# lRomul/ball-action-spotting

Measured on AMD Instinct MI355X. Metric: frame-windows/sec (fwd+bwd) at 15x736x1280, batch 4, higher is better.
Workload: dtype bf16; 1 GPU; sampling_weights_001: 4x15x736x1280 windows/GPU, fwd + focal loss + bwd + grad all-reduce + AdamW (mds.train fused focal loss / multi-tensor optimizer); global_batch=4, parallelism=dp1

## Files before the change

ball-action-spotting_amd/csrc/k_pw.hip:

```cpp
#include <stdlib.h>
#include "gemm.h"

#define PW_BM 128
#ifndef MDS_PW_GPRE3
#define MDS_PW_GPRE3 1
#endif
#define PW_BN 128
#define PW_SP 72

template <typename T> struct PwCfg;
template <> struct PwCfg<bf16_t> { static const int KC = 64, LD = 80; };
template <> struct PwCfg<float> { static const int KC = 32, LD = 40; };

template <typename T, int PRO, int WN, int BM, int TAIL, bool SPLIT = false, bool DEEP = false>
__global__ __launch_bounds__(256, (WN == 2 && BM == 128) || TAIL == 1 || SPLIT || DEEP ? 2 : 3) void pw_fwd_kernel(mds_pw_fwd_args a) {
  MDS_CHAIN_PRIO();
  static_assert(!DEEP || (TAIL != 1 && (PRO == MDS_PRO_NONE || PRO == MDS_PRO_GATE) && WN == 2 && BM == 64), "DEEP variants");
  static_assert(!SPLIT || (TAIL != 1 && (PRO == MDS_PRO_NONE || PRO == MDS_PRO_GATE) && WN == 2 && BM == 64), "SPLIT variants");
  constexpr bool POST = TAIL == 1, EPI = TAIL == 2;
  typedef typename Frag<T>::type frag_t;
  typedef Mma<T, EPI && sizeof(T) == 4 && MDS_EVAL_X3> MM;
  constexpr int KC = PwCfg<T>::KC, LD = PwCfg<T>::LD, VPR = KC / 8, RPP = 256 / VPR, NL = BM / RPP;
  constexpr int BN = 64 * WN, MFW = (WN == 2 ? BM / 32 : BM / 64), NLW = BN / RPP;
  MDS_DYN_SMEM(smem);
  T* xs = (T*)smem;
  T* ws = xs + BM * LD;
  constexpr bool STG = sizeof(T) == 2;
  T* stg = ws + BN * LD + (threadIdx.x >> 6) * 16 * PW_SP;

  const int tid = threadIdx.x, lane = tid & 63, wave = MDS_UNIFORM(tid >> 6);
  const int i = lane & 15, q = lane >> 4;
  const int wm = WN == 2 ? wave >> 1 : wave, wn = WN == 2 ? wave & 1 : 0;
  const long m0 = (long)blockIdx.x * BM;
  const int N = a.N;
  const int K = a.K;
  const int kper = SPLIT ? ((K + (int)gridDim.z * PwCfg<T>::KC - 1) / ((int)gridDim.z * PwCfg<T>::KC)) * PwCfg<T>::KC : K;
  const int KB = SPLIT ? (int)blockIdx.z * kper : 0;
  const int KE = SPLIT ? (KB + kper < K ? KB + kper : K) : K;
  const T* x = (const T*)a.x;
  const T* w = (const T*)a.w;
  T* y = (T*)a.y;
  const int svec = tid % VPR, srow = tid / VPR;
  int grow[NL];
  if (PRO == MDS_PRO_BN_SILU_GATE || PRO == MDS_PRO_GATE) {
    const long rpg = a.pro.rows_per_group;
#pragma unroll
    for (int l = 0; l < NL; ++l) {
      const long m = m0 + srow + RPP * l;
      grow[l] = (int)((m < a.M ? m : a.M - 1) / rpg);
    }
  }

  const T* xrow[NL];
  bool xok[NL];
#pragma unroll
  for (int l = 0; l < NL; ++l) {
    const long m = m0 + srow + RPP * l;
    xok[l] = m < a.M;
    xrow[l] = x + (xok[l] ? m : 0) * K + 8 * svec;
  }
  for (int n0 = blockIdx.y * BN; n0 < N; n0 += gridDim.y * BN) {
    int nfr = (N - n0 - 64 * wn) >> 4;
    nfr = nfr < 0 ? 0 : (nfr > 4 ? 4 : nfr);
    f32x4 acc[MFW][4];
#pragma unroll
    for (int mf = 0; mf < MFW; ++mf)
#pragma unroll
      for (int nf = 0; nf < 4; ++nf) acc[mf][nf] = (f32x4){0.f, 0.f, 0.f, 0.f};

    RawV4<T> rys[POST ? MFW : 1][4];
    float pb[4] = {0.f, 0.f, 0.f, 0.f};
    if (EPI && tid < BN && n0 + tid < N) { pb[0] = a.epi.scale[n0 + tid]; pb[1] = a.epi.shift[n0 + tid]; }
    if (POST) {
      if (tid < BN && n0 + tid < N) {
#pragma unroll
        for (int k = 0; k < 4; ++k) pb[k] = a.post.bn[(long)k * N + n0 + tid];
      }
      const int nfr_ = (N - n0 - 64 * wn) >> 4;
#pragma unroll
      for (int mf = 0; mf < (POST ? MFW : 1); ++mf) {
        const long m = m0 + 16 * MFW * wm + 16 * mf + i;
        const T* ysrow = (const T*)a.post.y + (m < a.M ? m : 0) * N + n0 + (nfr_ > 0 ? 64 * wn : 0) + 4 * q;
#pragma unroll
        for (int nf = 0; nf < 4; ++nf) rys[mf][nf].ld(ysrow + (nf < nfr_ ? 16 * nf : 0));
      }
    }

    constexpr int NS = DEEP ? 2 : 1;
    RawV8<T> rx[NS][NL], rw[NS][NLW];
    constexpr bool GATED = PRO == MDS_PRO_BN_SILU_GATE || PRO == MDS_PRO_GATE;
    constexpr bool GPRE = (PRO == MDS_PRO_GATE || (PRO == MDS_PRO_BN_SILU_GATE && MDS_PW_GPRE3)) && NL <= 2;
    float rg[NS][GPRE ? NL : 1][8];
    const T* wrow[NLW];
    bool wok[NLW];
#pragma unroll
    for (int l = 0; l < NLW; ++l) {
      const int n = n0 + srow + RPP * l;
      wok[l] = n < N;
      wrow[l] = w + (long)(wok[l] ? n : 0) * K + 8 * svec;
    }
    constexpr bool SPRE = PRO == MDS_PRO_BN_SILU_GATE && MDS_PW_GPRE3 && NL <= 2;
    float psc[SPRE ? 8 : 1], psh[SPRE ? 8 : 1];
    auto issue = [&](int kc, RawV8<T> (&tx)[NL], RawV8<T> (&tw)[NLW], float (&tg)[GPRE ? NL : 1][8]) {
      const bool kok = kc + 8 * svec < KE;
      if (DEEP) {
        const int ko = kok ? kc : -8 * svec;
#pragma unroll
        for (int l = 0; l < NL; ++l) {
          tx[l].ld(xrow[l] + ko);
          if (GPRE) load8f(a.pro.gate + (long)grow[l] * K + (kok ? kc + 8 * svec : 0), tg[l]);
        }
#pragma unroll
        for (int l = 0; l < NLW; ++l) tw[l].ld(wrow[l] + ko);
        return;
      }
      if (SPRE) {
        const int kp = kok ? kc + 8 * svec : 0;
        load8f(a.pro.scale + kp, (float (&)[8])psc); load8f(a.pro.shift + kp, (float (&)[8])psh);
      }
#pragma unroll
      for (int l = 0; l < NL; ++l) {
        if (xok[l] && kok) tx[l].ld(xrow[l] + kc); else tx[l].zero();
        if (GPRE) load8f(a.pro.gate + (long)grow[l] * K + (kok ? kc + 8 * svec : 0), tg[l]);
      }
#pragma unroll
      for (int l = 0; l < NLW; ++l) {
        if (wok[l] && kok) tw[l].ld(wrow[l] + kc); else tw[l].zero();
      }
    };
    auto chunk = [&](int kc, RawV8<T> (&tx)[NL], RawV8<T> (&tw)[NLW], float (&tg)[GPRE ? NL : 1][8]) {
      const int kk = kc + 8 * svec;
      const bool kin = kk < KE;
      __syncthreads();
      if (PRO == MDS_PRO_NONE) {
#pragma unroll
        for (int l = 0; l < NL; ++l) {
          if (DEEP && !(xok[l] && kin)) tx[l].zero();
          tx[l].st(xs + (srow + RPP * l) * LD + 8 * svec);
        }
      } else {
        float sc[8], sh[8];
        if (SPRE) {
#pragma unroll
          for (int j = 0; j < 8; ++j) { sc[j] = psc[SPRE ? j : 0]; sh[j] = psh[SPRE ? j : 0]; }
        } else if (PRO != MDS_PRO_GATE && kin) { load8f(a.pro.scale + kk, sc); load8f(a.pro.shift + kk, sh); }
#pragma unroll
        for (int l = 0; l < NL; ++l) {
          const int r = srow + RPP * l;
          const long m = m0 + r;
          float v[8];
          tx[l].get(v);
          if (m < a.M && kin) {
            if (PRO != MDS_PRO_GATE) {
#pragma unroll
              for (int j = 0; j < 8; ++j) {
                float z = v[j] * sc[j] + sh[j];
                v[j] = (PRO == MDS_PRO_AFFINE) ? z : siluf_(z);
              }
            }
            if (GPRE) {
#pragma unroll
              for (int j = 0; j < 8; ++j) v[j] *= tg[l][j];
            } else if (GATED) {
              float g[8];
              load8f(a.pro.gate + (long)grow[l] * K + kk, g);
#pragma unroll
              for (int j = 0; j < 8; ++j) v[j] *= g[j];
            }
          } else if (DEEP) {
#pragma unroll
            for (int j = 0; j < 8; ++j) v[j] = 0.f;
          }
          store8(xs + r * LD + 8 * svec, v);
        }
      }
#pragma unroll
      for (int l = 0; l < NLW; ++l) {
        if (DEEP && !(wok[l] && kin)) tw[l].zero();
        tw[l].st(ws + (srow + RPP * l) * LD + 8 * svec);
      }
      __syncthreads();
      if (DEEP) issue(kc + 2 * KC, tx, tw, tg);
      else if (kc + KC < KE) issue(kc + KC, tx, tw, tg);
      const int ksteps = (KE - kc >= KC) ? KC / 32 : ((KE - kc + 31) >> 5);
#pragma unroll
      for (int ks = 0; ks < KC / 32; ++ks) {
        if (DEEP || ks < ksteps) {
          typename MM::frag xf[MFW];
#pragma unroll
          for (int mf = 0; mf < MFW; ++mf) xf[mf] = MM::prep(ld_frag(xs + (16 * MFW * wm + 16 * mf + i) * LD + 32 * ks + 8 * q));
#pragma unroll
          for (int nf = 0; nf < 4; ++nf) {
            const typename MM::frag wf = MM::prep(ld_frag(ws + (64 * wn + 16 * nf + i) * LD + 32 * ks + 8 * q));
#pragma unroll
            for (int mf = 0; mf < MFW; ++mf) MM::mma(wf, xf[mf], acc[mf][nf]);
          }
        }
      }
    };
    if (!SPLIT || KB < KE) issue(KB, rx[0], rw[0], rg[0]);
    if (DEEP) {
      issue(KB + KC, rx[NS - 1], rw[NS - 1], rg[NS - 1]);
      for (int kc = KB; kc < KE; kc += 2 * KC) {
        chunk(kc, rx[0], rw[0], rg[0]);
        chunk(kc + KC, rx[NS - 1], rw[NS - 1], rg[NS - 1]);
      }
    } else {
      for (int kc = KB; kc < KE; kc += KC) chunk(kc, rx[0], rw[0], rg[0]);
    }
    if (SPLIT) {
      const long MN = a.M * (long)N;
#pragma unroll
      for (int mf = 0; mf < MFW; ++mf) {
        const long m = m0 + 16 * MFW * wm + 16 * mf + i;
        if (m < a.M) {
          float* prow = a.split_part + (long)blockIdx.z * MN + m * N + n0 + 64 * wn + 4 * q;
#pragma unroll
          for (int nf = 0; nf < 4; ++nf)
            if (nf < nfr) st_coherent4(prow + 16 * nf, acc[mf][nf]);
        }
      }
      int* lastp = (int*)smem;
      mds_wait_stores();
      __syncthreads();
      if (tid == 0) {
        int* tk = a.split_ticket + ((long)blockIdx.x * ((N + BN - 1) / BN) + n0 / BN) * MDS_PW_SPLIT_TICKET_STRIDE;
        const int t = atomicAdd(tk, 1);
        const int last = t == (int)gridDim.z - 1;
        if (last) atomicExch(tk, 0);
        *lastp = last;
      }
      __syncthreads();
      const bool last = *lastp != 0;
      __syncthreads();
      if (!last) continue;
#pragma unroll
      for (int mf = 0; mf < MFW; ++mf)
#pragma unroll
        for (int nf = 0; nf < 4; ++nf) acc[mf][nf] = (f32x4){0.f, 0.f, 0.f, 0.f};
      for (int z0 = 0; z0 < (int)gridDim.z; z0 += 4) {
        f32x4 t[4][MFW][4];
#pragma unroll
        for (int zz = 0; zz < 4; ++zz)
#pragma unroll
          for (int mf = 0; mf < MFW; ++mf) {
            const long m = m0 + 16 * MFW * wm + 16 * mf + i;
            const bool ok = m < a.M && z0 + zz < (int)gridDim.z;
            const float* prow = a.split_part + (long)(z0 + zz) * MN + m * N + n0 + 64 * wn + 4 * q;
#pragma unroll
            for (int nf = 0; nf < 4; ++nf) t[zz][mf][nf] = (ok && nf < nfr) ? ld_coherent4(prow + 16 * nf) : (f32x4){0.f, 0.f, 0.f, 0.f};
          }
#pragma unroll
        for (int zz = 0; zz < 4; ++zz)
#pragma unroll
          for (int mf = 0; mf < MFW; ++mf)
#pragma unroll
            for (int nf = 0; nf < 4; ++nf) acc[mf][nf] += t[zz][mf][nf];
      }
    }

    float ps[16], pss[16];
#pragma unroll
    for (int e = 0; e < 16; ++e) { ps[e] = 0.f; pss[e] = 0.f; }
    float* pbn = (float*)smem;
    if (POST) {
      __syncthreads();
      if (tid < BN) {
#pragma unroll
        for (int k = 0; k < 4; ++k) pbn[k * BN + tid] = pb[k];
      }
      __syncthreads();
    }
    if (EPI) {
      __syncthreads();
      if (tid < BN) { pbn[tid] = pb[0]; pbn[BN + tid] = pb[1]; }
      __syncthreads();
    }
#pragma unroll
    for (int mf = 0; mf < MFW; ++mf) {
      const long m = m0 + 16 * MFW * wm + 16 * mf + i;
      const bool ok = m < a.M;
      T* yrow = y + (ok ? m : 0) * N + n0 + 64 * wn + 4 * q;
      float v[4][4];
#pragma unroll
      for (int nf = 0; nf < 4; ++nf)
#pragma unroll
        for (int r = 0; r < 4; ++r) v[nf][r] = acc[mf][nf][r];
      if (EPI) {
#pragma unroll
        for (int nf = 0; nf < 4; ++nf) {
          const float* pc = pbn + 64 * wn + 16 * nf + 4 * q;
          const f32x4 sc = *(const f32x4*)pc, sh = *(const f32x4*)(pc + BN);
#pragma unroll
          for (int r = 0; r < 4; ++r) {
            const float z = v[nf][r] * sc[r] + sh[r];
            v[nf][r] = a.epi.mode == MDS_EPI_BN_SILU ? siluf_(z) : z;
          }
        }
      }
      if (a.residual && ok) {
        const T* rrow = (const T*)a.residual + m * N + n0 + 64 * wn + 4 * q;
#pragma unroll
        for (int nf = 0; nf < 4; ++nf) {
          if (nf < nfr) {
            float rr[4];
            load4(rrow + 16 * nf, rr);
#pragma unroll
            for (int r = 0; r < 4; ++r) v[nf][r] += rr[r];
          }
        }
      }
      if (POST) {
        const float mk = (a.post.mode == MDS_POST_MASK) ? a.post.mask[(unsigned)(ok ? m : 0) / (unsigned)a.post.rows_per_group] : 1.0f;
#pragma unroll
        for (int nf = 0; nf < 4; ++nf) {
          if (nf < nfr) {
            const float ys[4] = {rys[mf][nf].get(0), rys[mf][nf].get(1), rys[mf][nf].get(2), rys[mf][nf].get(3)};
            const float* pc = pbn + 64 * wn + 16 * nf + 4 * q;
            const f32x4 mu = *(const f32x4*)(pc + 2 * BN), rs = *(const f32x4*)(pc + 3 * BN);
            if (a.post.mode == MDS_POST_SILU) {
              const f32x4 sc = *(const f32x4*)pc, sh = *(const f32x4*)(pc + BN);
#pragma unroll
              for (int r = 0; r < 4; ++r) v[nf][r] *= silu_gradf_(ys[r] * sc[r] + sh[r]);
            }
#pragma unroll
            for (int r = 0; r < 4; ++r) {
              const float g = Elem<T>::rnd(v[nf][r]) * mk;
              ps[nf * 4 + r] += g;
              pss[nf * 4 + r] += g * ((ys[r] - mu[r]) * rs[r]);
            }
          }
        }
      }
      if (STG) {
#pragma unroll
        for (int nf = 0; nf < 4; ++nf) store4(stg + i * PW_SP + 16 * nf + 4 * q, v[nf]);
        wave_lds_sync();
        T* ybase = y + (m0 + 16 * MFW * wm + 16 * mf) * N + n0 + 64 * wn;
#pragma unroll
        for (int t = 0; t < 2; ++t) {
          const int vv = lane + 64 * t, row = vv >> 3, c = vv & 7;
          if (m0 + 16 * MFW * wm + 16 * mf + row < a.M && (c >> 1) < nfr) {
            RawV8<T> o;
            o.ld(stg + row * PW_SP + 8 * c);
            o.st(ybase + (long)row * N + 8 * c);
          }
        }
        wave_lds_sync();
      } else if (ok) {
#pragma unroll
        for (int nf = 0; nf < 4; ++nf)
          if (nf < nfr) store4(yrow + 16 * nf, v[nf]);
      }
      if (!POST) {
#pragma unroll
        for (int nf = 0; nf < 4; ++nf)
#pragma unroll
          for (int r = 0; r < 4; ++r) { ps[nf * 4 + r] += v[nf][r]; pss[nf * 4 + r] += v[nf][r] * v[nf][r]; }
      }
    }
    if (POST ? (a.post.stats != nullptr) : (a.stats != nullptr)) {
      const int e = reduce_scatter16(ps, i);
      reduce_scatter16(pss, i);
      const int n = n0 + 64 * wn + 16 * (e >> 2) + 4 * q + (e & 3);
      if (n < N) {
        const long so = (long)((blockIdx.x + wm) % MDS_STAT_SLOTS) * 2 * N;
        if (POST) {
          atomicAdd(a.post.stats + so + n, (double)ps[0]);
          atomicAdd(a.post.stats + so + N + n, (double)pss[0]);
        } else {
          atomicAdd(a.stats + so + n, (double)ps[0]);
          atomicAdd(a.stats + so + N + n, (double)pss[0]);
        }
      }
    }
  }
}

int pw_fwd_wres_try(const mds_pw_fwd_args* a, mds_stream_t stream);
int pw_fwd_k_try(const mds_pw_fwd_args* a, mds_stream_t stream);

int c3_pw_try(const mds_pw_fwd_args* a, mds_stream_t stream);

extern "C" int mds_pw_fwd(const mds_pw_fwd_args* a, mds_stream_t stream) {
  MDS_REQUIRE(a && a->M > 0 && a->K > 0 && a->N > 0, "pw_fwd: bad dims");
  MDS_REQUIRE(a->K % 8 == 0 && a->N % 16 == 0, "pw_fwd: K=%d must be a multiple of 8, N=%d of 16", a->K, a->N);
  MDS_REQUIRE(a->x && a->w && a->y, "pw_fwd: null pointer");
  MDS_REQUIRE(a->pro.mode == MDS_PRO_NONE || a->pro.mode == MDS_PRO_GATE || (a->pro.scale && a->pro.shift), "pw_fwd: prologue needs scale/shift");
  MDS_REQUIRE((a->pro.mode != MDS_PRO_BN_SILU_GATE && a->pro.mode != MDS_PRO_GATE) || (a->pro.gate && a->pro.rows_per_group > 0), "pw_fwd: gate prologue");
  const bool post = a->post.mode != MDS_POST_NONE;
  const bool epi = a->epi.mode != MDS_EPI_NONE;
  if (epi) {
    MDS_REQUIRE(a->epi.scale && a->epi.shift && !a->stats && !post, "pw_fwd: an output transform needs scale/shift and excludes statistics and post statistics");
    MDS_REQUIRE(a->pro.mode == MDS_PRO_NONE || a->pro.mode == MDS_PRO_GATE || a->pro.mode == MDS_PRO_BN_SILU, "pw_fwd: an output transform takes the NONE, GATE or BN_SILU prologue");
  }
  if (post) {
    MDS_REQUIRE(a->post.y && a->post.bn && a->post.stats && !a->stats, "pw_fwd: post statistics need y, bn, stats (and no forward stats)");
    MDS_REQUIRE(a->post.mode != MDS_POST_MASK || (a->post.mask && a->post.rows_per_group > 0), "pw_fwd: post mask");
    MDS_REQUIRE(a->pro.mode == MDS_PRO_NONE && a->M < 4294967295L, "pw_fwd: post statistics are a data-gradient feature (no forward prologue)");
  }
  const bool split = a->split > 1;
  if (split) {
    MDS_REQUIRE(a->split <= MDS_PW_MAX_SPLIT && a->split_part && a->split_ticket, "pw_fwd: split-K needs split <= %d, a partial buffer and tickets", MDS_PW_MAX_SPLIT);
    MDS_REQUIRE(!post && !a->stats && (a->pro.mode == MDS_PRO_NONE || a->pro.mode == MDS_PRO_GATE),
                "pw_fwd: split-K is an inference-plan feature (NONE / GATE prologue, no statistics, no post statistics)");
  }
  if (!split && c3_pw_try(a, stream)) return mds_check_launch("pw_fwd");
  if (!split) { const int rc = pw_fwd_k_try(a, stream); if (rc <= 0) return rc; }
  if (!split) { const int rc = pw_fwd_wres_try(a, stream); if (rc <= 0) return rc; }
  const int wn = (a->N <= 64 && !split) ? 1 : 2;
  const int BN = 64 * wn;
  const long bar64 = mds_knob(MDS_KNOB_PW_BM64) > 0 ? 1000L * mds_knob(MDS_KNOB_PW_BM64) : 400000;
  const int bm = (wn == 2 && a->M <= bar64) ? 64 : PW_BM;
  MDS_REQUIRE(!split || bm == 64, "pw_fwd: split-K is for small M (64-row tiles)");
  const int mt = cdiv(a->M, bm), nt = cdiv(a->N, BN);
  int gy = 1;
  if (nt > 1) { gy = cdiv(mds_knob(MDS_KNOB_PW_GY) > 0 ? mds_knob(MDS_KNOB_PW_GY) : 1536, mt); if (gy > nt) gy = nt; if (gy < 1) gy = 1; }
  dim3 grid(mt, gy, split ? a->split : 1), block(256);
  const int kchunks = cdiv(split ? cdiv(a->K, a->split) : a->K, PwCfg<float>::KC);
  const bool deep = a->dtype == MDS_F32 && (epi || split) && wn == 2 && bm == 64 && kchunks >= 3 &&
                    (long)mt * gy * (split ? a->split : 1) <= 256 && mds_knob(MDS_KNOB_PW_DEEP) != 1;
#define PW_GOSPLIT(T, PRO, TAIL_) \
  do { const size_t smem = (size_t)(bm + BN) * PwCfg<T>::LD * sizeof(T) + (sizeof(T) == 2 ? 4 * 16 * PW_SP * 2 : 0); \
       if (sizeof(T) == 4 && deep) MDS_LAUNCH((pw_fwd_kernel<T, PRO, 2, 64, TAIL_, true, sizeof(T) == 4>), grid, block, smem, stream, *a); \
       else MDS_LAUNCH((pw_fwd_kernel<T, PRO, 2, 64, TAIL_, true>), grid, block, smem, stream, *a); } while (0)
#define PW_GODEEP(T, PRO) \
  do { const size_t smem = (size_t)(bm + BN) * PwCfg<T>::LD * sizeof(T) + (sizeof(T) == 2 ? 4 * 16 * PW_SP * 2 : 0); \
       MDS_LAUNCH((pw_fwd_kernel<T, PRO, 2, 64, 2, false, sizeof(T) == 4>), grid, block, smem, stream, *a); } while (0)
#define PW_GO2(T, PRO, TAIL_) \
  do { const size_t smem = (size_t)(bm + BN) * PwCfg<T>::LD * sizeof(T) + (sizeof(T) == 2 ? 4 * 16 * PW_SP * 2 : 0); \
       if (wn == 2 && bm == 64) MDS_LAUNCH((pw_fwd_kernel<T, PRO, 2, 64, TAIL_>), grid, block, smem, stream, *a); \
       else if (wn == 2) MDS_LAUNCH((pw_fwd_kernel<T, PRO, 2, 128, TAIL_>), grid, block, smem, stream, *a); \
       else MDS_LAUNCH((pw_fwd_kernel<T, PRO, 1, 128, TAIL_>), grid, block, smem, stream, *a); } while (0)
#define PW_GO(T, PRO) PW_GO2(T, PRO, 0)
  MDS_DISPATCH_DTYPE(a->dtype, T, {
    if (split) {
      if (epi) { if (a->pro.mode == MDS_PRO_GATE) PW_GOSPLIT(T, MDS_PRO_GATE, 2); else PW_GOSPLIT(T, MDS_PRO_NONE, 2); }
      else { if (a->pro.mode == MDS_PRO_GATE) PW_GOSPLIT(T, MDS_PRO_GATE, 0); else PW_GOSPLIT(T, MDS_PRO_NONE, 0); }
    }
    else if (post) PW_GO2(T, MDS_PRO_NONE, 1);
    else if (epi && deep && sizeof(T) == 4 && (a->pro.mode == MDS_PRO_GATE || a->pro.mode == MDS_PRO_NONE)) {
      if (a->pro.mode == MDS_PRO_GATE) PW_GODEEP(T, MDS_PRO_GATE); else PW_GODEEP(T, MDS_PRO_NONE);
    }
    else if (epi) { if (a->pro.mode == MDS_PRO_GATE) PW_GO2(T, MDS_PRO_GATE, 2); else if (a->pro.mode == MDS_PRO_BN_SILU) PW_GO2(T, MDS_PRO_BN_SILU, 2); else PW_GO2(T, MDS_PRO_NONE, 2); }
    else switch (a->pro.mode) {
      case MDS_PRO_NONE: PW_GO(T, MDS_PRO_NONE); break;
      case MDS_PRO_AFFINE: PW_GO(T, MDS_PRO_AFFINE); break;
      case MDS_PRO_BN_SILU: PW_GO(T, MDS_PRO_BN_SILU); break;
      case MDS_PRO_BN_SILU_GATE: PW_GO(T, MDS_PRO_BN_SILU_GATE); break;
      case MDS_PRO_GATE: PW_GO(T, MDS_PRO_GATE); break;
      default: mds_set_error("pw_fwd: prologue mode %d", a->pro.mode); return MDS_ERR_BAD_ARG;
    }
  });
#undef PW_GO
#undef PW_GO2
#undef PW_GOSPLIT
#undef PW_GODEEP
  return mds_check_launch("pw_fwd");
}

extern "C" int mds_pw_fwd_split(long M, int K, int N, int dtype) {
  const int knob = mds_knob(MDS_KNOB_PW_SPLIT);
  if (knob == 1 || M <= 0 || K <= 0 || N <= 0) return 1;
  const int kc = dtype == MDS_BF16 ? PwCfg<bf16_t>::KC : PwCfg<float>::KC;
  const long chunks = cdiv(K, kc), tiles = cdiv(M, MDS_PW_SPLIT_TILE_ROWS) * cdiv(N, 128);
  if (tiles >= 100 || chunks < 16) return 1;
  long s = knob >= 2 ? knob : 4;
  if (s > chunks / 3) s = chunks / 3;
  if (s > MDS_PW_MAX_SPLIT) s = MDS_PW_MAX_SPLIT;
  return s < 2 ? 1 : (int)s;
}

#define WG_ROWS 64
template <typename T> struct WgCfg;
template <> struct WgCfg<float> { static const int MW = 1, LDT = WG_ROWS + 4; };
template <int LDT> MDS_DEV int wg_off(int c, int m) { return c * LDT + 8 * ((m >> 3) ^ ((c >> 3) & 7)) + (m & 7); }
MDS_DEV void wg_put(float* base, int off, float v0, float) { base[off] = v0; }

template <typename T, int PRO, int NF, int KF>
__global__ __launch_bounds__(256, 2) void pw_wgrad_kernel(mds_pw_wgrad_args a, int rows_per_block) {
  typedef typename Frag<T>::type frag_t;
  constexpr int MW = WgCfg<T>::MW, LDT = WgCfg<T>::LDT;
  constexpr int NT = 64 * NF, KT = 16 * KF, XCH = KT / 8, YCH = NT / 8;
  constexpr int XN = (WG_ROWS / MW) * XCH, YN = (WG_ROWS / MW) * YCH;
  constexpr int XI = (XN + 255) / 256, YI = (YN + 255) / 256;
  MDS_DYN_SMEM(smem);
  T* xsT = (T*)smem;
  T* dsT = xsT + KT * LDT;
  const int tid = threadIdx.x, lane = tid & 63, wave = MDS_UNIFORM(tid >> 6);
  const int i = lane & 15, q = lane >> 4;
  const int K = a.K, N = a.N;
  const int ntiles_k = (K + KT - 1) / KT;
  const int n0 = (blockIdx.y / ntiles_k) * NT, kt0 = (blockIdx.y % ntiles_k) * KT;
  const long mbeg = (long)blockIdx.x * rows_per_block;
  long mend = mbeg + rows_per_block;
  if (mend > a.M) mend = a.M;
  const T* x = (const T*)a.x;
  const T* dy = (const T*)a.dy;
  const int kfr = (K - kt0 >= KT) ? KF : ((K - kt0 + 15) >> 4);
  const bool det = a.partial.buf != nullptr;
  float* const dw = wg_base(a.dw, a.partial, (long)N * K, blockIdx.x);

  constexpr bool FIXED_CH = (256 % XCH) == 0;
  float sc[8], sh[8];
  if (FIXED_CH && PRO != MDS_PRO_NONE && PRO != MDS_PRO_GATE) {
    const int kx = kt0 + 8 * (tid % XCH);
    if (kx < K) { load8f(a.pro.scale + kx, sc); load8f(a.pro.shift + kx, sh); }
  }

  f32x4 acc[NF][KF];
#pragma unroll
  for (int u = 0; u < NF; ++u)
#pragma unroll
    for (int v = 0; v < KF; ++v) acc[u][v] = (f32x4){0.f, 0.f, 0.f, 0.f};

  RawV8<T> rx[XI][MW], ry[YI][MW];
  auto issue = [&](long mb) {
#pragma unroll
    for (int p = 0; p < XI; ++p) {
      const int it = tid + 256 * p, kx = kt0 + 8 * (it % XCH);
#pragma unroll
      for (int h = 0; h < MW; ++h) {
        const long m = mb + (it / XCH) * MW + h;
        if (it < XN && m < mend && kx < K) rx[p][h].ld(x + m * K + kx); else rx[p][h].zero();
      }
    }
#pragma unroll
    for (int p = 0; p < YI; ++p) {
      const int it = tid + 256 * p, n = n0 + 8 * (it % YCH);
#pragma unroll
      for (int h = 0; h < MW; ++h) {
        const long m = mb + (it / YCH) * MW + h;
        if (it < YN && m < mend && n < N) ry[p][h].ld(dy + m * N + n); else ry[p][h].zero();
      }
    }
  };
  issue(mbeg);
  for (long mb = mbeg; mb < mend; mb += WG_ROWS) {
    __syncthreads();
#pragma unroll
    for (int p = 0; p < XI; ++p) {
      const int it = tid + 256 * p, xc = it % XCH, kx = kt0 + 8 * xc;
      if (it < XN) {
        float v[MW][8];
#pragma unroll
        for (int h = 0; h < MW; ++h) {
          const long m = mb + (it / XCH) * MW + h;
          rx[p][h].get(v[h]);
          if (PRO != MDS_PRO_NONE && m < mend && kx < K) {
            if (PRO != MDS_PRO_GATE) {
              float scl[8], shl[8];
              if (!FIXED_CH) { load8f(a.pro.scale + kx, scl); load8f(a.pro.shift + kx, shl); }
#pragma unroll
              for (int j = 0; j < 8; ++j) {
                float z = v[h][j] * (FIXED_CH ? sc[j] : scl[j]) + (FIXED_CH ? sh[j] : shl[j]);
                v[h][j] = (PRO == MDS_PRO_AFFINE) ? z : siluf_(z);
              }
            }
            if (PRO == MDS_PRO_BN_SILU_GATE || PRO == MDS_PRO_GATE) {
              float g[8];
              load8f(a.pro.gate + (long)((unsigned)m / (unsigned)a.pro.rows_per_group) * K + kx, g);
#pragma unroll
              for (int j = 0; j < 8; ++j) v[h][j] *= g[j];
            }
          }
        }
        const int ml = (it / XCH) * MW;
#pragma unroll
        for (int j = 0; j < 8; ++j) wg_put(xsT, wg_off<LDT>(8 * xc + j, ml), v[0][j], v[MW - 1][j]);
      }
    }
#pragma unroll
    for (int p = 0; p < YI; ++p) {
      const int it = tid + 256 * p;
      if (it < YN) {
        float v[MW][8];
#pragma unroll
        for (int h = 0; h < MW; ++h) {
          ry[p][h].get(v[h]);
        }
        const int ml = (it / YCH) * MW, yc = it % YCH;
#pragma unroll
        for (int j = 0; j < 8; ++j) wg_put(dsT, wg_off<LDT>(8 * yc + j, ml), v[0][j], v[MW - 1][j]);
      }
    }
    __syncthreads();
    if (mb + WG_ROWS < mend) issue(mb + WG_ROWS);
#pragma unroll
    for (int ks = 0; ks < WG_ROWS / 32; ++ks) {
      const int g = 4 * ks + q;
      frag_t yf[NF];
#pragma unroll
      for (int u = 0; u < NF; ++u) {
        const int c = 16 * (NF * wave + u) + i;
        yf[u] = ld_frag(dsT + c * LDT + 8 * (g ^ ((c >> 3) & 7)));
      }
#pragma unroll
      for (int v = 0; v < KF; ++v) {
        if (v < kfr) {
          const int c = 16 * v + i;
          const frag_t xf = ld_frag(xsT + c * LDT + 8 * (g ^ ((c >> 3) & 7)));
#pragma unroll
          for (int u = 0; u < NF; ++u) mma16(yf[u], xf, acc[u][v]);
        }
      }
    }
  }
#pragma unroll
  for (int u = 0; u < NF; ++u)
#pragma unroll
    for (int v = 0; v < KF; ++v) {
      const int k = kt0 + 16 * v + i;
#pragma unroll
      for (int r = 0; r < 4; ++r) {
        const int n = n0 + 16 * (NF * wave + u) + 4 * q + r;
        if (n < N && k < K) wg_out(dw + (long)n * K + k, acc[u][v][r], det);
      }
    }
}

template <int PRO, int NF, int KF>
__global__ __launch_bounds__(256, 2) void pw_wgrad_tr_kernel(mds_pw_wgrad_args a, int rows_per_block, int dbg) {
  typedef bf16_t T;
  constexpr int NT = 64 * NF, KT = 16 * KF, XCH = KT / 8, YCH = NT / 8;
  constexpr int LDX = KT + 16, LDY = NT + 16;
  constexpr int XN = WG_ROWS * XCH, YN = WG_ROWS * YCH;
  constexpr int XI = (XN + 255) / 256, YI = (YN + 255) / 256;
  MDS_DYN_SMEM(smem);
  T* xs = (T*)smem;
  T* ds = xs + WG_ROWS * LDX;
  const int tid = threadIdx.x, lane = tid & 63, wave = MDS_UNIFORM(tid >> 6);
  const int i = lane & 15, q = lane >> 4;
  const int K = a.K, N = a.N;
  const int ntiles_k = (K + KT - 1) / KT;
  const int ntiles = ntiles_k * ((N + NT - 1) / NT), slot = blockIdx.x >> 3;
  const int tile_id = slot % ntiles, split_id = (int)(blockIdx.x & 7) + 8 * (slot / ntiles);
  const int n0 = (tile_id / ntiles_k) * NT, kt0 = (tile_id % ntiles_k) * KT;
  const long mbeg = (long)split_id * rows_per_block;
  long mend = mbeg + rows_per_block;
  if (mend > a.M) mend = a.M;
  if (mbeg >= a.M) return;
  const bool det = a.partial.buf != nullptr;
  float* const dw = wg_base(a.dw, a.partial, (long)a.N * a.K, split_id);
  const T* x = (const T*)a.x;
  const T* dy = (const T*)a.dy;
  const int kfr = (K - kt0 >= KT) ? KF : ((K - kt0 + 15) >> 4);
  constexpr bool FIXED_CH = (256 % XCH) == 0;
  float sc[8], sh[8];
  if (FIXED_CH && PRO != MDS_PRO_NONE && PRO != MDS_PRO_GATE) {
    const int kx = kt0 + 8 * (tid % XCH);
    if (kx < K) { load8f(a.pro.scale + kx, sc); load8f(a.pro.shift + kx, sh); }
  }
  f32x4 acc[NF][KF];
#pragma unroll
  for (int u = 0; u < NF; ++u)
#pragma unroll
    for (int v = 0; v < KF; ++v) acc[u][v] = (f32x4){0.f, 0.f, 0.f, 0.f};

  RawV8<T> rx[XI], ry[YI];
  int xr[XI], yr[YI];
  bool xok[XI], yok[YI];
  const T* px[XI];
  const T* py[YI];
#pragma unroll
  for (int p = 0; p < XI; ++p) {
    const int it = tid + 256 * p, kx = kt0 + 8 * (it % XCH);
    xr[p] = it / XCH;
    xok[p] = it < XN && kx < K;
    px[p] = x + (mbeg + xr[p]) * K + (xok[p] ? kx : 0);
  }
#pragma unroll
  for (int p = 0; p < YI; ++p) {
    const int it = tid + 256 * p, n = n0 + 8 * (it % YCH);
    yr[p] = it / YCH;
    yok[p] = it < YN && n < N;
    py[p] = dy + (mbeg + yr[p]) * N + (yok[p] ? n : 0);
  }
  const long xstep = (long)WG_ROWS * K, ystep = (long)WG_ROWS * N;
  constexpr bool GATED = PRO == MDS_PRO_BN_SILU_GATE || PRO == MDS_PRO_GATE;
  float rg[GATED ? XI : 1][8];
  auto issue = [&](long mb) {
    const int left = (int)(mend - mb);
#pragma unroll
    for (int p = 0; p < XI; ++p) {
      if (xok[p] && xr[p] < left) rx[p].ld(px[p]); else rx[p].zero();
      px[p] += xstep;
      if (GATED) {
        const long m = mb + xr[p];
        const int kx = kt0 + 8 * ((tid + 256 * p) % XCH);
        load8f(a.pro.gate + (long)((unsigned)(m < mend ? m : mbeg) / (unsigned)a.pro.rows_per_group) * K + (kx < K ? kx : 0), rg[p]);
      }
    }
#pragma unroll
    for (int p = 0; p < YI; ++p) {
      if (yok[p] && yr[p] < left) ry[p].ld(py[p]); else ry[p].zero();
      py[p] += ystep;
    }
  };
  issue(mbeg);
  const int ra = 16 * (q >> 1) + 4 * (q & 1);
  const int lrow = (i >> 2), lcol = 4 * (i & 3);
  for (long mb = mbeg; mb < mend; mb += WG_ROWS) {
    __syncthreads();
#pragma unroll
    for (int p = 0; p < XI; ++p) {
      const int it = tid + 256 * p, xc = it % XCH, kx = kt0 + 8 * xc, ml = it / XCH;
      if (it < XN) {
        if (PRO == MDS_PRO_NONE) {
          rx[p].st(xs + ml * LDX + 8 * xc);
        } else {
          const long m = mb + ml;
          float v[8];
          rx[p].get(v);
          if (m < mend && kx < K) {
            if (PRO != MDS_PRO_GATE) {
              float scl[8], shl[8];
              if (!FIXED_CH) { load8f(a.pro.scale + kx, scl); load8f(a.pro.shift + kx, shl); }
// ... 131 lines not shown
```

include/mds.h:

```cpp
#ifndef MDS_H
#define MDS_H
#ifdef __cplusplus
extern "C" {
#endif

#define MDS_VERSION 142
#define MDS_F32 0
#define MDS_BF16 1
#define MDS_STAT_SLOTS 32

#define MDS_ERR_BAD_ARG (-1)
#define MDS_ERR_UNSUPPORTED (-2)
#define MDS_ERR_LAUNCH (-3)

typedef void* mds_stream_t;

int mds_version(void);
const char* mds_last_error(void);
#define MDS_KNOB_CONV_BLOCKS 0
#define MDS_KNOB_DW_ORDER 1
#define MDS_KNOB_PW_WRES 2
#define MDS_KNOB_WG_DBG 4
#define MDS_KNOB_WG_BLOCKS 5
#define MDS_KNOB_DW3_L 7
#define MDS_KNOB_STREAM_BLOCKS 8
#define MDS_KNOB_DW2_L 9
#define MDS_KNOB_PW_SPLIT 10
#define MDS_KNOB_DW2_R 11
#define MDS_KNOB_PW_GY 12
#define MDS_KNOB_PW_BM64 13
#define MDS_KNOB_REDUCE_PASSES 14
#define MDS_KNOB_DW2_BLOCKS 15
#define MDS_KNOB_REDUCE_BLOCKS 16
#define MDS_KNOB_PW_DEEP 17
#define MDS_KNOB_PWK 18
#define MDS_KNOB_PWK_BM 19
#define MDS_KNOB_STEM_FWD 20
#define MDS_KNOB_DW3G 21
#define MDS_KNOB_C3 22
#define MDS_KNOB_C3_BWD_BLOCKS 24
#define MDS_KNOB_COUNT 25
int mds_dev_set(int knob, int value);
int mds_launch_event(void* event);

typedef struct {
  float* buf;
  long floats;
} mds_partial_t;
#define MDS_FINISH_GROUPS 4
#define MDS_FINISH_GROUPS_MID 16
#define MDS_FINISH_GROUPS_SMALL 64
#define MDS_FINISH_WIDE 65536
#define MDS_FINISH_MID 4096
typedef struct {
  const float* partial;
  float* dst;
  long numel;
  long slots;
  long slot_stride;
} mds_wgrad_finish_args;
long mds_wgrad_finish(const mds_wgrad_finish_args* a, mds_stream_t stream);

typedef struct {
  float* mask;
  const float* keep;
  long n;
  unsigned long long seed;
  unsigned long long draw;
  unsigned int stream;
  int keep_checked;
} mds_mask_fill_args;
long mds_mask_fill(const mds_mask_fill_args* a, mds_stream_t stream);

#define MDS_EPI_NONE 0
#define MDS_EPI_AFFINE 1
#define MDS_EPI_BN_SILU 2
typedef struct {
  int mode;
  const float* scale;
  const float* shift;
} mds_epi_t;

#define MDS_PRO_NONE 0
#define MDS_PRO_AFFINE 1
#define MDS_PRO_BN_SILU 2
#define MDS_PRO_BN_SILU_GATE 3
#define MDS_PRO_GATE 4
typedef struct {
  int mode;
  const float* scale;
  const float* shift;
  const float* gate;
  long rows_per_group;
} mds_pro_t;

#define MDS_G_PLAIN 0
#define MDS_G_SILU 1
#define MDS_G_SE_SILU 2
#define MDS_G_MASK 3
typedef struct {
  int mode;
  const void* u;
  const float* gate;
  const float* dpooled;
  const float* mask;
  long rows_per_group;
} mds_gsrc_t;

typedef struct {
  int mode;
  mds_gsrc_t g;
  const void* y;
  const float* bn;
  const float* lin;
} mds_dyp_t;

#define MDS_POST_NONE 0
#define MDS_POST_PLAIN 1
#define MDS_POST_MASK 2
#define MDS_POST_SILU 3
typedef struct {
  int mode;
  const void* y;
  const float* bn;
  const float* mask;
  long rows_per_group;
  double* stats;
} mds_poststat_t;

typedef struct {
  int dtype;
  long M;
  int K, N;
  const void* x;
  const void* w;
  void* y;
  mds_pro_t pro;
  const void* residual;
  double* stats;
  mds_poststat_t post;
  mds_epi_t epi;
  const void* w_frag;
  int split;
  float* split_part;
  int* split_ticket;
  int form;
} mds_pw_fwd_args;
int mds_pw_fwd(const mds_pw_fwd_args* a, mds_stream_t stream);
int mds_pw_fwd_split(long M, int K, int N, int dtype);
int mds_pw_fwd_wants_frag(long M, int K, int N, int dtype, int data_gradient);
#define MDS_PW_MAX_SPLIT 16
#define MDS_PW_SPLIT_TILE_ROWS 64
#define MDS_PW_SPLIT_TICKET_STRIDE 32

typedef struct {
  int dtype;
  long M;
  int K, N;
  const void* x;
  const void* dy;
  float* dw;
  mds_pro_t pro;
  mds_partial_t partial;
} mds_pw_wgrad_args;
int mds_pw_wgrad(const mds_pw_wgrad_args* a, mds_stream_t stream);
long mds_pw_wgrad_partial_floats(const mds_pw_wgrad_args* a);

#define MDS_PROJECT_CIN_MAX 48
#define MDS_PROJECT_MID_MAX 256
#define MDS_PROJECT_COUT_MAX 48
typedef struct {
  const void* w;
  int cout;
  const float* scale;
  const float* shift;
} mds_project_t;

#define MDS_MAX_TAPS 9
typedef struct {
  int dtype;
  int N, IH, IW, Cin;
  int OH, OW, Cout;
  int A, B;
  int oy0, ox0, os;
  int is;
  int ntaps;
  int dy[MDS_MAX_TAPS], dx[MDS_MAX_TAPS], wi[MDS_MAX_TAPS];
  int wtaps;
  const void* x;
  const void* w;
  void* y;
  mds_pro_t pro;
  const void* residual;
  double* stats;
  int ngroups;
  int g_ntaps[4], g_oy0[4], g_ox0[4], g_A[4], g_B[4];
  mds_epi_t epi;
  mds_poststat_t post;
  mds_project_t project;
} mds_conv_fwd_args;
int mds_conv_fwd(const mds_conv_fwd_args* a, mds_stream_t stream);
int mds_conv_dgrad_post_ok(int dtype, int N, int IH, int IW, int Cin, int Cout, int stride, int has_residual);

typedef struct {
  int dtype;
  int N, IH, IW, Cin, OH, OW, Cout;
  int is, ntaps;
  int dy[MDS_MAX_TAPS], dx[MDS_MAX_TAPS], wi[MDS_MAX_TAPS];
  int wtaps;
  const void* x;
  const void* dyt;
  float* dw;
  mds_pro_t pro;
  mds_partial_t partial;
} mds_conv_wgrad_args;
int mds_conv_wgrad(const mds_conv_wgrad_args* a, mds_stream_t stream);
long mds_conv_wgrad_partial_floats(const mds_conv_wgrad_args* a);

typedef struct {
  const unsigned char* u8;
  int nsrc, src_h, src_w;
  int pad_top, pad_left;
  float scale;
} mds_ingest_t;
typedef struct {
  int dtype;
  int N, H, W, OH, OW, Cout;
  int pad_t, pad_l;
  const float* x;
  const void* w;
  void* y;
  double* stats;
  mds_ingest_t ingest;
  mds_epi_t epi;
} mds_stem_fwd_args;
int mds_stem_fwd(const mds_stem_fwd_args* a, mds_stream_t stream);

typedef struct {
  int dtype;
  int N, H, W, OH, OW, Cout;
  int pad_t, pad_l;
  const float* x;
  const void* dy;
  float* dw;
  mds_dyp_t dyp;
  mds_partial_t partial;
} mds_stem_wgrad_args;
int mds_stem_wgrad(const mds_stem_wgrad_args* a, mds_stream_t stream);
long mds_stem_wgrad_partial_floats(const mds_stem_wgrad_args* a);

typedef struct {
  int dtype;
  int N, H, W, OH, OW, Cout;
  int pad_t, pad_l;
  const void* w;
  const void* dy;
  float* dx;
  mds_dyp_t dyp;
} mds_stem_dgrad_args;
long mds_stem_dgrad(const mds_stem_dgrad_args* a, mds_stream_t stream);

typedef struct {
  const void* x;
  const void* w;
  int cin;
  const float* scale;
  const float* shift;
} mds_expand_t;

#define MDS_SE_TAIL_CMAX 1280
#define MDS_SE_TAIL_RMAX 64
typedef struct {
  int R;
  const float* w1;
  const float* b1;
  const float* w2t;
  const float* b2;
  float* hidden;
  float* gate;
  int* ticket;
} mds_se_tail_t;

typedef struct {
  int dtype;
  int N, T, IH, IW, C;
  int OH, OW;
  int stride, pad_t, pad_l;
  int kt;
  const void* x;
  const float* w;
  void* y;
  mds_pro_t pro;
  double* stats;
  mds_epi_t epi;
  double* pool;
  float pool_inv;
  mds_expand_t expand;
  mds_se_tail_t se;
} mds_dw_fwd_args;
int mds_dw_fwd(const mds_dw_fwd_args* a, mds_stream_t stream);

typedef struct {
  int dtype;
  int N, T, IH, IW, C, OH, OW;
  int stride, pad_t, pad_l, kt;
  const void* x;
  const void* dy;
  const float* w;
  void* g;
  float* dw;
  mds_pro_t pro;
  const float* mean;
  const float* rstd;
  double* stats;
  mds_partial_t partial;
} mds_dw_bwd_args;
int mds_dw_bwd(const mds_dw_bwd_args* a, mds_stream_t stream);
long mds_dw_bwd_partial_floats(const mds_dw_bwd_args* a);

typedef struct {
  int C;
  long count;
  const double* stats;
  const float* gamma;
  const float* beta;
  float eps, momentum;
  int training;
  float* running_mean;
  float* running_var;
  long long* num_batches_tracked;
  float* out;
} mds_bn_finalize_args;
int mds_bn_finalize(const mds_bn_finalize_args* a, mds_stream_t stream);

typedef struct {
  const float* gamma;
  const float* beta;
  const float* running_mean;
  const float* running_var;
  float* out;
  float eps;
  int C;
// ... 427 lines not shown
```

Baseline: 336.4 frame-windows/s.

## Add whole-N 192-column tile variant for bf16 pointwise conv forward

Adds a WN=3 template variant of the pointwise forward GEMM in which each block covers the full N (up to 192 columns), with six 16-column fragments per wave, so the activation tile is loaded once per block rather than once per N tile. The dispatcher picks it for bf16 layers with 128<N<=192 when there are enough M tiles to fill the CUs, and a new knob can force it on or off. The staging pitch, the epilogue stores and the per-channel statistic reductions are generalized for the extra columns. In exchange the wider accumulator raises register pressure and lowers occupancy to two blocks per CU, and the extra statistics handling adds more atomics.

```diff
diff --git a/ball-action-spotting_amd/csrc/k_pw.hip b/ball-action-spotting_amd/csrc/k_pw.hip
--- a/ball-action-spotting_amd/csrc/k_pw.hip
+++ b/ball-action-spotting_amd/csrc/k_pw.hip
@@ -12,25 +12,38 @@
 template <> struct PwCfg<bf16_t> { static const int KC = 64, LD = 80; };
 template <> struct PwCfg<float> { static const int KC = 32, LD = 40; };
 
+MDS_DEV int reduce_scatter8(float (&vals)[8], int i) {
+#pragma unroll
+  for (int k = 0; k < 8; ++k) vals[k] += __shfl_xor(vals[k], 8);
+  reduce_scatter_step<4, 4>(vals, (i & 4) != 0);
+  reduce_scatter_step<2, 2>(vals, (i & 2) != 0);
+  reduce_scatter_step<1, 1>(vals, (i & 1) != 0);
+  return ((i & 4) ? 4 : 0) + ((i & 2) ? 2 : 0) + ((i & 1) ? 1 : 0);
+}
+
 template <typename T, int PRO, int WN, int BM, int TAIL, bool SPLIT = false, bool DEEP = false>
-__global__ __launch_bounds__(256, (WN == 2 && BM == 128) || TAIL == 1 || SPLIT || DEEP ? 2 : 3) void pw_fwd_kernel(mds_pw_fwd_args a) {
+__global__ __launch_bounds__(256, (WN == 2 && BM == 128) || WN == 3 || TAIL == 1 || SPLIT || DEEP ? 2 : 3) void pw_fwd_kernel(mds_pw_fwd_args a) {
   MDS_CHAIN_PRIO();
   static_assert(!DEEP || (TAIL != 1 && (PRO == MDS_PRO_NONE || PRO == MDS_PRO_GATE) && WN == 2 && BM == 64), "DEEP variants");
+  static_assert(WN != 3 || (sizeof(T) == 2 && BM == 64 && TAIL != 2 && !SPLIT && !DEEP), "whole-N tile variants");
   static_assert(!SPLIT || (TAIL != 1 && (PRO == MDS_PRO_NONE || PRO == MDS_PRO_GATE) && WN == 2 && BM == 64), "SPLIT variants");
   constexpr bool POST = TAIL == 1, EPI = TAIL == 2;
   typedef typename Frag<T>::type frag_t;
   typedef Mma<T, EPI && sizeof(T) == 4 && MDS_EVAL_X3> MM;
   constexpr int KC = PwCfg<T>::KC, LD = PwCfg<T>::LD, VPR = KC / 8, RPP = 256 / VPR, NL = BM / RPP;
-  constexpr int BN = 64 * WN, MFW = (WN == 2 ? BM / 32 : BM / 64), NLW = BN / RPP;
+  constexpr int BN = 64 * WN, MFW = (WN >= 2 ? BM / 32 : BM / 64), NLW = BN / RPP;
+  constexpr int NFW = WN == 3 ? 6 : 4, CW = 16 * NFW;
   MDS_DYN_SMEM(smem);
   T* xs = (T*)smem;
   T* ws = xs + BM * LD;
   constexpr bool STG = sizeof(T) == 2;
-  T* stg = ws + BN * LD + (threadIdx.x >> 6) * 16 * PW_SP;
+  constexpr int SP = CW + 8;
+  static_assert(NFW != 4 || SP == PW_SP, "staging pitch of the 64-column waves");
+  T* stg = ws + BN * LD + (threadIdx.x >> 6) * 16 * SP;
 
   const int tid = threadIdx.x, lane = tid & 63, wave = MDS_UNIFORM(tid >> 6);
   const int i = lane & 15, q = lane >> 4;
-  const int wm = WN == 2 ? wave >> 1 : wave, wn = WN == 2 ? wave & 1 : 0;
+  const int wm = WN >= 2 ? wave >> 1 : wave, wn = WN >= 2 ? wave & 1 : 0;
   const long m0 = (long)blockIdx.x * BM;
   const int N = a.N;
   const int K = a.K;
@@ -60,15 +73,15 @@
     xrow[l] = x + (xok[l] ? m : 0) * K + 8 * svec;
   }
   for (int n0 = blockIdx.y * BN; n0 < N; n0 += gridDim.y * BN) {
-    int nfr = (N - n0 - 64 * wn) >> 4;
-    nfr = nfr < 0 ? 0 : (nfr > 4 ? 4 : nfr);
-    f32x4 acc[MFW][4];
+    int nfr = (N - n0 - CW * wn) >> 4;
+    nfr = nfr < 0 ? 0 : (nfr > NFW ? NFW : nfr);
+    f32x4 acc[MFW][NFW];
 #pragma unroll
     for (int mf = 0; mf < MFW; ++mf)
 #pragma unroll
-      for (int nf = 0; nf < 4; ++nf) acc[mf][nf] = (f32x4){0.f, 0.f, 0.f, 0.f};
-
-    RawV4<T> rys[POST ? MFW : 1][4];
+      for (int nf = 0; nf < NFW; ++nf) acc[mf][nf] = (f32x4){0.f, 0.f, 0.f, 0.f};
+
+    RawV4<T> rys[POST ? MFW : 1][NFW];
     float pb[4] = {0.f, 0.f, 0.f, 0.f};
     if (EPI && tid < BN && n0 + tid < N) { pb[0] = a.epi.scale[n0 + tid]; pb[1] = a.epi.shift[n0 + tid]; }
     if (POST) {
@@ -76,13 +89,13 @@
 #pragma unroll
         for (int k = 0; k < 4; ++k) pb[k] = a.post.bn[(long)k * N + n0 + tid];
       }
-      const int nfr_ = (N - n0 - 64 * wn) >> 4;
+      const int nfr_ = (N - n0 - CW * wn) >> 4;
 #pragma unroll
       for (int mf = 0; mf < (POST ? MFW : 1); ++mf) {
         const long m = m0 + 16 * MFW * wm + 16 * mf + i;
-        const T* ysrow = (const T*)a.post.y + (m < a.M ? m : 0) * N + n0 + (nfr_ > 0 ? 64 * wn : 0) + 4 * q;
-#pragma unroll
-        for (int nf = 0; nf < 4; ++nf) rys[mf][nf].ld(ysrow + (nf < nfr_ ? 16 * nf : 0));
+        const T* ysrow = (const T*)a.post.y + (m < a.M ? m : 0) * N + n0 + (nfr_ > 0 ? CW * wn : 0) + 4 * q;
+#pragma unroll
+        for (int nf = 0; nf < NFW; ++nf) rys[mf][nf].ld(ysrow + (nf < nfr_ ? 16 * nf : 0));
       }
     }
 
@@ -190,8 +203,8 @@
 #pragma unroll
           for (int mf = 0; mf < MFW; ++mf) xf[mf] = MM::prep(ld_frag(xs + (16 * MFW * wm + 16 * mf + i) * LD + 32 * ks + 8 * q));
 #pragma unroll
-          for (int nf = 0; nf < 4; ++nf) {
-            const typename MM::frag wf = MM::prep(ld_frag(ws + (64 * wn + 16 * nf + i) * LD + 32 * ks + 8 * q));
+          for (int nf = 0; nf < NFW; ++nf) {
+            const typename MM::frag wf = MM::prep(ld_frag(ws + (CW * wn + 16 * nf + i) * LD + 32 * ks + 8 * q));
 #pragma unroll
             for (int mf = 0; mf < MFW; ++mf) MM::mma(wf, xf[mf], acc[mf][nf]);
           }
@@ -260,8 +273,11 @@
     }
 
     float ps[16], pss[16];
+    float ps2[NFW > 4 ? 8 : 1], pss2[NFW > 4 ? 8 : 1];
 #pragma unroll
     for (int e = 0; e < 16; ++e) { ps[e] = 0.f; pss[e] = 0.f; }
+#pragma unroll
+    for (int e = 0; e < (NFW > 4 ? 8 : 1); ++e) { ps2[e] = 0.f; pss2[e] = 0.f; }
     float* pbn = (float*)smem;
     if (POST) {
       __syncthreads();
@@ -280,16 +296,16 @@
     for (int mf = 0; mf < MFW; ++mf) {
       const long m = m0 + 16 * MFW * wm + 16 * mf + i;
       const bool ok = m < a.M;
-      T* yrow = y + (ok ? m : 0) * N + n0 + 64 * wn + 4 * q;
-      float v[4][4];
-#pragma unroll
-      for (int nf = 0; nf < 4; ++nf)
+      T* yrow = y + (ok ? m : 0) * N + n0 + CW * wn + 4 * q;
+      float v[NFW][4];
+#pragma unroll
+      for (int nf = 0; nf < NFW; ++nf)
 #pragma unroll
         for (int r = 0; r < 4; ++r) v[nf][r] = acc[mf][nf][r];
       if (EPI) {
 #pragma unroll
-        for (int nf = 0; nf < 4; ++nf) {
-          const float* pc = pbn + 64 * wn + 16 * nf + 4 * q;
+        for (int nf = 0; nf < NFW; ++nf) {
+          const float* pc = pbn + CW * wn + 16 * nf + 4 * q;
           const f32x4 sc = *(const f32x4*)pc, sh = *(const f32x4*)(pc + BN);
 #pragma unroll
           for (int r = 0; r < 4; ++r) {
@@ -299,9 +315,9 @@
         }
       }
       if (a.residual && ok) {
-        const T* rrow = (const T*)a.residual + m * N + n0 + 64 * wn + 4 * q;
-#pragma unroll
-        for (int nf = 0; nf < 4; ++nf) {
+        const T* rrow = (const T*)a.residual + m * N + n0 + CW * wn + 4 * q;
+#pragma unroll
+        for (int nf = 0; nf < NFW; ++nf) {
           if (nf < nfr) {
             float rr[4];
             load4(rrow + 16 * nf, rr);
@@ -313,10 +329,10 @@
       if (POST) {
         const float mk = (a.post.mode == MDS_POST_MASK) ? a.post.mask[(unsigned)(ok ? m : 0) / (unsigned)a.post.rows_per_group] : 1.0f;
 #pragma unroll
-        for (int nf = 0; nf < 4; ++nf) {
+        for (int nf = 0; nf < NFW; ++nf) {
           if (nf < nfr) {
             const float ys[4] = {rys[mf][nf].get(0), rys[mf][nf].get(1), rys[mf][nf].get(2), rys[mf][nf].get(3)};
-            const float* pc = pbn + 64 * wn + 16 * nf + 4 * q;
+            const float* pc = pbn + CW * wn + 16 * nf + 4 * q;
             const f32x4 mu = *(const f32x4*)(pc + 2 * BN), rs = *(const f32x4*)(pc + 3 * BN);
             if (a.post.mode == MDS_POST_SILU) {
               const f32x4 sc = *(const f32x4*)pc, sh = *(const f32x4*)(pc + BN);
@@ -326,43 +342,50 @@
 #pragma unroll
             for (int r = 0; r < 4; ++r) {
               const float g = Elem<T>::rnd(v[nf][r]) * mk;
-              ps[nf * 4 + r] += g;
-              pss[nf * 4 + r] += g * ((ys[r] - mu[r]) * rs[r]);
+              float& s1 = nf < 4 ? ps[(nf & 3) * 4 + r] : ps2[NFW > 4 ? (nf & 1) * 4 + r : 0];
+              float& s2 = nf < 4 ? pss[(nf & 3) * 4 + r] : pss2[NFW > 4 ? (nf & 1) * 4 + r : 0];
+              s1 += g;
+              s2 += g * ((ys[r] - mu[r]) * rs[r]);
             }
           }
         }
       }
       if (STG) {
 #pragma unroll
-        for (int nf = 0; nf < 4; ++nf) store4(stg + i * PW_SP + 16 * nf + 4 * q, v[nf]);
+        for (int nf = 0; nf < NFW; ++nf) store4(stg + i * SP + 16 * nf + 4 * q, v[nf]);
         wave_lds_sync();
-        T* ybase = y + (m0 + 16 * MFW * wm + 16 * mf) * N + n0 + 64 * wn;
-#pragma unroll
-        for (int t = 0; t < 2; ++t) {
-          const int vv = lane + 64 * t, row = vv >> 3, c = vv & 7;
+        T* ybase = y + (m0 + 16 * MFW * wm + 16 * mf) * N + n0 + CW * wn;
+        constexpr int VR = 2 * NFW;
+#pragma unroll
+        for (int t = 0; t < VR / 4; ++t) {
+          const int vv = lane + 64 * t, row = vv / VR, c = vv % VR;
           if (m0 + 16 * MFW * wm + 16 * mf + row < a.M && (c >> 1) < nfr) {
             RawV8<T> o;
-            o.ld(stg + row * PW_SP + 8 * c);
+            o.ld(stg + row * SP + 8 * c);
             o.st(ybase + (long)row * N + 8 * c);
           }
         }
         wave_lds_sync();
       } else if (ok) {
 #pragma unroll
-        for (int nf = 0; nf < 4; ++nf)
+        for (int nf = 0; nf < NFW; ++nf)
           if (nf < nfr) store4(yrow + 16 * nf, v[nf]);
       }
       if (!POST) {
 #pragma unroll
-        for (int nf = 0; nf < 4; ++nf)
-#pragma unroll
-          for (int r = 0; r < 4; ++r) { ps[nf * 4 + r] += v[nf][r]; pss[nf * 4 + r] += v[nf][r] * v[nf][r]; }
+        for (int nf = 0; nf < NFW; ++nf)
+#pragma unroll
+          for (int r = 0; r < 4; ++r) {
+            float& s1 = nf < 4 ? ps[(nf & 3) * 4 + r] : ps2[NFW > 4 ? (nf & 1) * 4 + r : 0];
+            float& s2 = nf < 4 ? pss[(nf & 3) * 4 + r] : pss2[NFW > 4 ? (nf & 1) * 4 + r : 0];
+            s1 += v[nf][r]; s2 += v[nf][r] * v[nf][r];
+          }
       }
     }
     if (POST ? (a.post.stats != nullptr) : (a.stats != nullptr)) {
       const int e = reduce_scatter16(ps, i);
       reduce_scatter16(pss, i);
-      const int n = n0 + 64 * wn + 16 * (e >> 2) + 4 * q + (e & 3);
+      const int n = n0 + CW * wn + 16 * (e >> 2) + 4 * q + (e & 3);
       if (n < N) {
         const long so = (long)((blockIdx.x + wm) % MDS_STAT_SLOTS) * 2 * N;
         if (POST) {
@@ -371,6 +394,17 @@
         } else {
           atomicAdd(a.stats + so + n, (double)ps[0]);
           atomicAdd(a.stats + so + N + n, (double)pss[0]);
+        }
+      }
+      if constexpr (NFW > 4) {
+        const int e2 = reduce_scatter8(ps2, i);
+        reduce_scatter8(pss2, i);
+        const int n2 = n0 + CW * wn + 64 + 16 * (e2 >> 2) + 4 * q + (e2 & 3);
+        if (i < 8 && n2 < N) {
+          const long so = (long)((blockIdx.x + wm) % MDS_STAT_SLOTS) * 2 * N;
+          double* sl = POST ? a.post.stats : a.stats;
+          atomicAdd(sl + so + n2, (double)ps2[0]);
+          atomicAdd(sl + so + N + n2, (double)pss2[0]);
         }
       }
     }
@@ -413,6 +447,19 @@
   const long bar64 = mds_knob(MDS_KNOB_PW_BM64) > 0 ? 1000L * mds_knob(MDS_KNOB_PW_BM64) : 400000;
   const int bm = (wn == 2 && a->M <= bar64) ? 64 : PW_BM;
   MDS_REQUIRE(!split || bm == 64, "pw_fwd: split-K is for small M (64-row tiles)");
+  const int wide_knob = mds_knob(MDS_KNOB_PW_WIDE);
+  const bool wide_dg = a->form ? a->form == 2 : (post || a->residual != nullptr);
+  const bool wide = a->dtype == MDS_BF16 && !split && !epi && a->N > 128 && a->N <= 192 && bm == 64 && wide_knob != 1 &&
+                    (a->pro.mode == MDS_PRO_NONE || (a->pro.mode == MDS_PRO_BN_SILU_GATE && !post)) &&
+                    (wide_knob == 2 || (cdiv(a->M, 64) >= mds_cu_count() && (!wide_dg || wide_knob == 3)));
+  if (wide) {
+    dim3 grid(cdiv(a->M, 64), 1, 1), block(256);
+    const size_t smem = (size_t)(64 + 192) * PwCfg<bf16_t>::LD * sizeof(bf16_t) + 4 * 16 * (96 + 8) * sizeof(bf16_t);
+    if (post) MDS_LAUNCH((pw_fwd_kernel<bf16_t, MDS_PRO_NONE, 3, 64, 1>), grid, block, smem, stream, *a);
+    else if (a->pro.mode == MDS_PRO_NONE) MDS_LAUNCH((pw_fwd_kernel<bf16_t, MDS_PRO_NONE, 3, 64, 0>), grid, block, smem, stream, *a);
+    else MDS_LAUNCH((pw_fwd_kernel<bf16_t, MDS_PRO_BN_SILU_GATE, 3, 64, 0>), grid, block, smem, stream, *a);
+    return mds_check_launch("pw_fwd");
+  }
   const int mt = cdiv(a->M, bm), nt = cdiv(a->N, BN);
   int gy = 1;
   if (nt > 1) { gy = cdiv(mds_knob(MDS_KNOB_PW_GY) > 0 ? mds_knob(MDS_KNOB_PW_GY) : 1536, mt); if (gy > nt) gy = nt; if (gy < 1) gy = 1; }
diff --git a/include/mds.h b/include/mds.h
--- a/include/mds.h
+++ b/include/mds.h
@@ -38,6 +38,7 @@
 #define MDS_KNOB_STEM_FWD 20
 #define MDS_KNOB_DW3G 21
 #define MDS_KNOB_C3 22
+#define MDS_KNOB_PW_WIDE 23
 #define MDS_KNOB_C3_BWD_BLOCKS 24
 #define MDS_KNOB_COUNT 25
 int mds_dev_set(int knob, int value);
```

After: 335.5 frame-windows/s. Within noise of the previous version (-0.3%).
